# xuyuan/waymo_2d_tracking

Hardware: AMD Instinct MI355X
Metric: end-to-end frames/sec (detect+SORT) on 1920x1280 Waymo frames (higher is better)
Workload: dtype f32; 1 GPU; Cascade R-CNN X152-32x8d-FPN dconv (random-init, fp32, batch 1) on synthetic 1920x1280x3 frames -> top-100 detections/frame -> SORT (max_age 2, min_hits 0, all boxes tracked; trackers resident for the whole segment); 5 cameras x 2 frames per step per GPU; 1x1 and dense 3x3 convolutions: f32 operands as exact 3 x bf16 splits, six cross terms on the bf16 matrix cores, f32 accumulate (csrc/det_gemm_s; stage=e2e, parallelism=sequence-shard x1

## Files before the change

waymo_2d_tracking_amd/csrc/det_gemm_split.hip:

```cpp
#include "common.h"
#include "../../include/waymodet.h"
#include <cstdlib>
#include <cstring>

namespace {

using bf16x8 = __attribute__((ext_vector_type(8))) __bf16;
using bf16x2 = __attribute__((ext_vector_type(2))) __bf16;
using f32x2 = __attribute__((ext_vector_type(2))) float;
using f32x16 = __attribute__((ext_vector_type(16))) float;
using u32x4 = __attribute__((ext_vector_type(4))) unsigned;

constexpr int BK = 64;
constexpr int BN = 256;
constexpr int NTHREADS = 512;
constexpr int CHUNK = 6144;

struct SplitArgs {
    const float* a;
    const unsigned char* ap;
    const uint4* w;
    const float* bias;
    const float* residual;
    const unsigned char* resp;
    float* out;
    unsigned char* outp;
    long lda, ldc;
    int M, N, K, relu;
    int tiles_m, tiles_n;
    int splitk;
    float* part;
    long long* stamps;
    int H, W, C, Ho, Wo, stride, pad, ksize;
};

__device__ __forceinline__ unsigned pk_bf16(float a, float b) {
    const f32x2 v = {a, b};
    return __builtin_bit_cast(unsigned, __builtin_convertvector(v, bf16x2));
}

__device__ __forceinline__ void split_pair(float x0, float x1, unsigned& h, unsigned& m, unsigned& l) {
    h = pk_bf16(x0, x1);
    const float r0 = x0 - __uint_as_float(h << 16), r1 = x1 - __uint_as_float(h & 0xffff0000u);
    m = pk_bf16(r0, r1);
    const float s0 = r0 - __uint_as_float(m << 16), s1 = r1 - __uint_as_float(m & 0xffff0000u);
    l = pk_bf16(s0, s1);
}

__device__ __forceinline__ float bf_lo(unsigned v) { return __uint_as_float(v << 16); }
__device__ __forceinline__ float bf_hi(unsigned v) { return __uint_as_float(v & 0xffff0000u); }

__device__ __forceinline__ size_t planes_offset(int row, int col, int ncols) {
    return ((size_t)(row >> 5) * (size_t)(ncols >> 5) + (size_t)(col >> 5)) * CHUNK +
           (size_t)((row & 31) * 64 + ((((col >> 3) & 3) ^ ((row >> 2) & 3)) << 4) + ((col >> 2) & 1) * 8);
}

constexpr int LDC = BN + 8;

template <int MT>
__device__ __forceinline__ void split_epilogue(const SplitArgs& p, unsigned char* smem, const f32x16 (&acc)[MT], int m0, int n0, int wave, int lane, int mlim,
                                               int row_mul = 1, int row_add = 0) {
    const int rr = lane & 31, rg = lane >> 5;
    float* ct = reinterpret_cast<float*>(smem);
    const int ncols = p.N - n0 < BN ? p.N - n0 : BN;
    constexpr int PASS = 3;
    auto stage = [&](int i0) {
        if (i0 > 0) __builtin_amdgcn_s_barrier();
#pragma unroll
        for (int i = i0; i < i0 + PASS && i < MT; ++i)
#pragma unroll
            for (int e = 0; e < 16; ++e)
                ct[((i - i0) * 32 + (e & 3) + 8 * (e >> 2) + 4 * rg) * LDC + 32 * wave + rr] = acc[i][e];
        __builtin_amdgcn_s_waitcnt(0xC07F);
        __builtin_amdgcn_s_barrier();
    };
    if (p.outp == nullptr) {
        const int c4 = 4 * lane;
        float4 bv = make_float4(0.f, 0.f, 0.f, 0.f);
        if (p.bias && c4 < ncols) bv = *reinterpret_cast<const float4*>(p.bias + n0 + c4);
        constexpr int RPW = 32 * PASS / 8;
#pragma unroll
        for (int i0 = 0; i0 < MT; i0 += PASS) {
            const int nrows = 32 * ((MT - i0) < PASS ? (MT - i0) : PASS);
            float4 rv[RPW];
            if (p.residual) {
#pragma unroll
                for (int j = 0; j < RPW; ++j) {
                    const int r = wave + 8 * j, row = m0 + 32 * i0 + r;
                    rv[j] = make_float4(0.f, 0.f, 0.f, 0.f);
                    if (r < nrows && row < mlim && c4 < ncols)
                        rv[j] = *reinterpret_cast<const float4*>(p.residual + (size_t)(row * row_mul + row_add) * p.ldc + n0 + c4);
                }
            } else if (p.resp) {
#pragma unroll
                for (int j = 0; j < RPW; ++j) {
                    const int r = wave + 8 * j, row = m0 + 32 * i0 + r;
                    rv[j] = make_float4(0.f, 0.f, 0.f, 0.f);
                    if (r < nrows && row < mlim && c4 < ncols) {
                        const unsigned char* q = p.resp + planes_offset(row * row_mul + row_add, n0 + c4, p.N);
                        const uint2 h = *reinterpret_cast<const uint2*>(q), m = *reinterpret_cast<const uint2*>(q + 2048),
                                    l = *reinterpret_cast<const uint2*>(q + 4096);
                        rv[j] = make_float4((bf_lo(h.x) + bf_lo(m.x)) + bf_lo(l.x), (bf_hi(h.x) + bf_hi(m.x)) + bf_hi(l.x),
                                            (bf_lo(h.y) + bf_lo(m.y)) + bf_lo(l.y), (bf_hi(h.y) + bf_hi(m.y)) + bf_hi(l.y));
                    }
                }
            }
            stage(i0);
#pragma unroll
            for (int j = 0; j < RPW; ++j) {
                const int r = wave + 8 * j, row = m0 + 32 * i0 + r;
                if (r < nrows && row < mlim && c4 < ncols) {
                    float4 v = *reinterpret_cast<const float4*>(ct + r * LDC + c4);
                    v.x += bv.x; v.y += bv.y; v.z += bv.z; v.w += bv.w;
                    if (p.residual || p.resp) { v.x += rv[j].x; v.y += rv[j].y; v.z += rv[j].z; v.w += rv[j].w; }
                    if (p.relu) { v.x = fmaxf(v.x, 0.f); v.y = fmaxf(v.y, 0.f); v.z = fmaxf(v.z, 0.f); v.w = fmaxf(v.w, 0.f); }
                    *reinterpret_cast<float4*>(p.out + (size_t)(row * row_mul + row_add) * p.ldc + n0 + c4) = v;
                }
            }
        }
        return;
    }
    const int ur = lane >> 2;
    constexpr int UPW = PASS * 8 * 2 / 8;
    const int ncb = ncols >> 5;
#pragma unroll
    for (int i0 = 0; i0 < MT; i0 += PASS) {
        const int nrb = (MT - i0) < PASS ? (MT - i0) : PASS;
        const int nunits = nrb * ncb * 2;
        uint4 rq[UPW][3];
#pragma unroll
        for (int j = 0; j < UPW; ++j) {
            const int u = wave + 8 * j;
            rq[j][0] = rq[j][1] = rq[j][2] = make_uint4(0u, 0u, 0u, 0u);
            if (u < nunits && m0 + 32 * (i0 + u / (2 * ncb)) < mlim) {
                const int rbi = u / (2 * ncb), cb = (u >> 1) - rbi * ncb, h = u & 1;
                const int r = 16 * h + ur, row = m0 + 32 * (i0 + rbi) + r;
                const int c8 = 8 * ((lane & 3) ^ ((r >> 2) & 3)), col = n0 + 32 * cb + c8;
                if (p.resp) {
                    const unsigned char* q = p.resp + ((size_t)(row >> 5) * (size_t)(p.N >> 5) + (size_t)(col >> 5)) * CHUNK + h * 1024 + lane * 16;
                    rq[j][0] = *reinterpret_cast<const uint4*>(q);
                    rq[j][1] = *reinterpret_cast<const uint4*>(q + 2048);
                    rq[j][2] = *reinterpret_cast<const uint4*>(q + 4096);
                } else if (p.residual && row < mlim) {
                    const uint4* q = reinterpret_cast<const uint4*>(p.residual + (size_t)row * p.ldc + col);
                    rq[j][0] = q[0];
                    rq[j][1] = q[1];
                }
            }
        }
        stage(i0);
#pragma unroll
        for (int j = 0; j < UPW; ++j) {
            const int u = wave + 8 * j;
            if (u < nunits && m0 + 32 * (i0 + u / (2 * ncb)) < mlim) {
                const int rbi = u / (2 * ncb), cb = (u >> 1) - rbi * ncb, h = u & 1;
                const int r = 16 * h + ur, row = m0 + 32 * (i0 + rbi) + r;
                const int c8 = 8 * ((lane & 3) ^ ((r >> 2) & 3)), col = n0 + 32 * cb + c8;
                const float* src = ct + (32 * rbi + r) * LDC + 32 * cb + c8;
                float4 v0 = *reinterpret_cast<const float4*>(src), v1 = *reinterpret_cast<const float4*>(src + 4);
                if (p.bias) {
                    const float4 b0 = *reinterpret_cast<const float4*>(p.bias + col), b1 = *reinterpret_cast<const float4*>(p.bias + col + 4);
                    v0.x += b0.x; v0.y += b0.y; v0.z += b0.z; v0.w += b0.w; v1.x += b1.x; v1.y += b1.y; v1.z += b1.z; v1.w += b1.w;
                }
                if (p.resp) {
                    const uint4 hh = rq[j][0], mm = rq[j][1], ll = rq[j][2];
                    v0.x += (bf_lo(hh.x) + bf_lo(mm.x)) + bf_lo(ll.x); v0.y += (bf_hi(hh.x) + bf_hi(mm.x)) + bf_hi(ll.x);
                    v0.z += (bf_lo(hh.y) + bf_lo(mm.y)) + bf_lo(ll.y); v0.w += (bf_hi(hh.y) + bf_hi(mm.y)) + bf_hi(ll.y);
                    v1.x += (bf_lo(hh.z) + bf_lo(mm.z)) + bf_lo(ll.z); v1.y += (bf_hi(hh.z) + bf_hi(mm.z)) + bf_hi(ll.z);
                    v1.z += (bf_lo(hh.w) + bf_lo(mm.w)) + bf_lo(ll.w); v1.w += (bf_hi(hh.w) + bf_hi(mm.w)) + bf_hi(ll.w);
                } else if (p.residual) {
                    const uint4 q0 = rq[j][0], q1 = rq[j][1];
                    v0.x += __uint_as_float(q0.x); v0.y += __uint_as_float(q0.y); v0.z += __uint_as_float(q0.z); v0.w += __uint_as_float(q0.w);
                    v1.x += __uint_as_float(q1.x); v1.y += __uint_as_float(q1.y); v1.z += __uint_as_float(q1.z); v1.w += __uint_as_float(q1.w);
                }
                if (p.relu) {
                    v0.x = fmaxf(v0.x, 0.f); v0.y = fmaxf(v0.y, 0.f); v0.z = fmaxf(v0.z, 0.f); v0.w = fmaxf(v0.w, 0.f);
                    v1.x = fmaxf(v1.x, 0.f); v1.y = fmaxf(v1.y, 0.f); v1.z = fmaxf(v1.z, 0.f); v1.w = fmaxf(v1.w, 0.f);
                }
                if (p.out && row < mlim) {
                    float4* d = reinterpret_cast<float4*>(p.out + (size_t)row * p.ldc + col);
                    d[0] = v0; d[1] = v1;
                }
                unsigned hv[4], mv[4], lv[4];
                split_pair(v0.x, v0.y, hv[0], mv[0], lv[0]); split_pair(v0.z, v0.w, hv[1], mv[1], lv[1]);
                split_pair(v1.x, v1.y, hv[2], mv[2], lv[2]); split_pair(v1.z, v1.w, hv[3], mv[3], lv[3]);
                unsigned char* q = p.outp + ((size_t)(row >> 5) * (size_t)(p.N >> 5) + (size_t)(col >> 5)) * CHUNK + h * 1024 + lane * 16;
                *reinterpret_cast<uint4*>(q) = make_uint4(hv[0], hv[1], hv[2], hv[3]);
                *reinterpret_cast<uint4*>(q + 2048) = make_uint4(mv[0], mv[1], mv[2], mv[3]);
                *reinterpret_cast<uint4*>(q + 4096) = make_uint4(lv[0], lv[1], lv[2], lv[3]);
            }
        }
    }
}

__device__ __forceinline__ int xcd_tile_id(int total) {
    const int x = blockIdx.x & 7, j = blockIdx.x >> 3;
    const int q = total >> 3, r = total & 7;
    if (j >= q + (x < r ? 1 : 0)) return -1;
    return (x < r ? x * (q + 1) : r * (q + 1) + (x - r) * q) + j;
}

template <int MT, int MODE>
__global__ __launch_bounds__(NTHREADS, 2) void gemm_split_kernel(const SplitArgs p) {
    extern __shared__ __attribute__((aligned(16))) unsigned char smem[];
    constexpr int BM = 32 * MT;
    constexpr int PLANE = BM * 64;
    constexpr int BUF = 3 * PLANE;
    const int tid = threadIdx.x, lane = tid & 63;
    const int wave = __builtin_amdgcn_readfirstlane(tid >> 6);
    constexpr bool CONV = MODE == 1 || MODE == 3;
    constexpr bool PM = MODE == 3;
    int id = PM ? (int)blockIdx.x : xcd_tile_id(p.tiles_m * p.tiles_n * p.splitk);
    if (id < 0 || (PM && id >= p.tiles_m * p.tiles_n)) return;
#ifdef WD_DEBUG
    long long t_start = 0, r_start = 0, t_main = 0, t_epi = 0;
    if (p.stamps) { t_start = __builtin_amdgcn_s_memtime(); r_start = __builtin_amdgcn_s_memrealtime(); }
    const int id_stamp = id;
#endif
    const int kz = PM ? 0 : id % p.splitk;
    if (!PM) id /= p.splitk;
    const int tm = id / p.tiles_n, tn = id - tm * p.tiles_n;
    int m0 = tm * BM;
    const int n0 = tn * BN;
    const int kc = CONV ? p.C / 32 : 1;
    int pm_y = 0, pm_x = 0, pm_nvt = 9;
    unsigned long long pm_taps = 0x876543210ull;
    if (PM) {
        const int nch = (p.M / (p.H * p.W) + BM - 1) / BM;
        const int wi = p.W - 2, hi = p.H - 2, ni = wi * hi, ne = 2 * wi + 2 * hi;
        int t = tm, c, q;
        if (t < ni * nch) { c = t / ni; q = t - c * ni; pm_y = 1 + q / wi; pm_x = 1 + q - (q / wi) * wi; }
        else if (t < (ni + ne) * nch) {
            t -= ni * nch; c = t / ne; q = t - c * ne;
            if (q < wi) { pm_y = 0; pm_x = 1 + q; }
            else if (q < 2 * wi) { pm_y = p.H - 1; pm_x = 1 + q - wi; }
            else if (q < 2 * wi + hi) { pm_x = 0; pm_y = 1 + q - 2 * wi; }
            else { pm_x = p.W - 1; pm_y = 1 + q - 2 * wi - hi; }
        } else { t -= (ni + ne) * nch; c = t >> 2; q = t & 3; pm_y = (q >> 1) ? p.H - 1 : 0; pm_x = (q & 1) ? p.W - 1 : 0; }
        m0 = c * BM;
        pm_taps = 0; pm_nvt = 0;
        for (int tp = 0; tp < 9; ++tp) {
            const int yy = pm_y + tp / 3 - 1, xx = pm_x + tp % 3 - 1;
            if (yy >= 0 && yy < p.H && xx >= 0 && xx < p.W) { pm_taps |= (unsigned long long)tp << (4 * pm_nvt); ++pm_nvt; }
        }
    }
    auto pm_tap = [&](int i) { return (int)((pm_taps >> (4 * i)) & 15ull); };
    const int nk_all = PM ? pm_nvt * kc : p.K / 32;
    const int per = (nk_all + p.splitk - 1) / p.splitk;
    const int k0 = kz * per;
    const int nk = (k0 + per <= nk_all) ? per : nk_all - k0;

    const int srow = tid >> 4, sk2 = tid & 15;
    unsigned aoff[MT];
    unsigned vmask[MT];
#pragma unroll
    for (int i = 0; i < MT; ++i) {
        int m = m0 + srow + 32 * i;
        if (PM) {
            const int maps = p.M / (p.H * p.W);
            m = m < maps ? m : maps - 1;
            aoff[i] = (unsigned)(((m * p.H + pm_y - 1) * p.W + pm_x - 1) * p.C + 2 * sk2);
            vmask[i] = 0x1ffu;
            continue;
        }
        m = m < p.M ? m : p.M - 1;
        if (MODE == 0) {
            aoff[i] = (unsigned)(m * p.lda) + 2u * sk2;
            vmask[i] = 1u;
        } else {
            const int hw = p.Ho * p.Wo;
            const int b = m / hw, rem = m - b * hw;
            const int yo = rem / p.Wo, xo = rem - yo * p.Wo;
            const int y0 = yo * p.stride - p.pad, x0 = xo * p.stride - p.pad;
            aoff[i] = (unsigned)(((b * p.H + y0) * p.W + x0) * p.C + 2 * sk2);
            unsigned vm = 0;
            for (int t = 0; t < p.ksize * p.ksize; ++t) {
                const int yy = y0 + t / p.ksize, xx = x0 + t % p.ksize;
                if (yy >= 0 && yy < p.H && xx >= 0 && xx < p.W) vm |= 1u << t;
            }
            vmask[i] = vm;
        }
    }
    float2 araw[MT];
    auto a_fetch = [&](int kt, int i) -> float2 {
        kt = k0 + (kt < nk ? kt : nk - 1);
        if (MODE == 0) {
            return *reinterpret_cast<const float2*>(p.a + (size_t)(aoff[i] + (unsigned)(kt * 32)));
        } else {
            const int ti = kt / kc, cb = kt - ti * kc;
            const int tap = PM ? pm_tap(ti) : ti;
            const int dy = tap / p.ksize, dx = tap - dy * p.ksize;
            const unsigned delta = (unsigned)((dy * p.W + dx) * p.C + cb * 32);
            const bool ok = ((vmask[i] >> tap) & 1u) != 0;
            const unsigned off = ok ? aoff[i] + delta : 2u * sk2;
            const float2 v = *reinterpret_cast<const float2*>(p.a + (size_t)off);
            return ok ? v : make_float2(0.f, 0.f);
        }
    };
    auto a_load_row = [&](int kt, int i) { araw[i] = a_fetch(kt, i); };
    int f_idx = 0, f_tap = 0, f_cb = 0;
    unsigned f_delta = 0;
    int f_act = 0;
    auto f_place = [&]() {
        f_act = PM ? pm_tap(f_tap) : f_tap;
        const int dy = p.ksize == 3 ? (f_act * 11) >> 5 : 0, dx = f_act - dy * p.ksize;
        f_delta = (unsigned)((dy * p.W + dx) * p.C + f_cb * 32);
    };
    auto f_set = [&](int kt) {
        f_idx = kt < nk ? kt : nk - 1;
        const int ks = k0 + f_idx;
        f_tap = ks / kc; f_cb = ks - f_tap * kc;
        f_place();
    };
    auto f_advance = [&](int kt) {
        if (kt < nk && kt > f_idx) {
            ++f_idx;
            if (++f_cb == kc) { f_cb = 0; ++f_tap; }
            f_place();
        }
    };
    auto a_fetch_cur = [&](int i) -> float2 {
        const bool ok = ((vmask[i] >> f_act) & 1u) != 0;
        const unsigned off = ok ? aoff[i] + f_delta : 2u * sk2;
        const float2 v = *reinterpret_cast<const float2*>(p.a + (size_t)off);
        return ok ? v : make_float2(0.f, 0.f);
    };
    const int wofs = srow * 64 + ((((sk2 >> 2) ^ ((srow >> 2) & 3))) << 4) + ((sk2 & 3) << 2);
    auto a_store_val = [&](int bufoff, int i, float2 v) {
        unsigned char* base = smem + bufoff + wofs + i * 2048;
        unsigned h, m, l;
        split_pair(v.x, v.y, h, m, l);
        *reinterpret_cast<unsigned*>(base) = h;
        *reinterpret_cast<unsigned*>(base + PLANE) = m;
        *reinterpret_cast<unsigned*>(base + 2 * PLANE) = l;
    };
    auto a_store_row = [&](int bufoff, int i) { a_store_val(bufoff, i, araw[i]); };

    const int nt32 = (n0 >> 5) + wave;
    const bool active = nt32 * 32 < p.N;
    const uint4* wbase = p.w + (size_t)(active ? nt32 : 0) * (size_t)(p.K / 16) * 192 + lane;
    const int nsub = nk * 2;
    bf16x8 wf[2][3];
    auto w_load = [&](int sub, int slot) {
        sub = 2 * k0 + (sub < nsub ? sub : nsub - 1);
        if (PM) {
            const int ti = sub / (2 * kc);
            sub = pm_tap(ti) * 2 * kc + (sub - ti * 2 * kc);
        }
        const uint4* q = wbase + (size_t)sub * 192;
#pragma unroll
        for (int pl = 0; pl < 3; ++pl) wf[slot][pl] = __builtin_bit_cast(bf16x8, q[pl * 64]);
    };

    f32x16 acc[MT];
#pragma unroll
    for (int i = 0; i < MT; ++i)
#pragma unroll
        for (int e = 0; e < 16; ++e) acc[i][e] = 0.f;

    const int rr = lane & 31, rg = lane >> 5;
    const int rofs0 = rr * 64 + ((((0 + rg) ^ ((rr >> 2) & 3))) << 4);
    const int rofs1 = rr * 64 + ((((2 + rg) ^ ((rr >> 2) & 3))) << 4);

    {
        float2 p0[MT], p1[MT];
#pragma unroll
        for (int i = 0; i < MT; ++i) p0[i] = a_fetch(0, i);
        w_load(0, 0);
        w_load(1, 1);
#pragma unroll
        for (int i = 0; i < MT; ++i) p1[i] = a_fetch(1, i);
#pragma unroll
        for (int i = 0; i < MT; ++i) a_load_row(2, i);
#pragma unroll
        for (int i = 0; i < MT; ++i) a_store_val(0, i, p0[i]);
#pragma unroll
        for (int i = 0; i < MT; ++i) a_store_val(BUF, i, p1[i]);
    }
    float2 aahead[MT];
#pragma unroll
    for (int i = 0; i < MT; ++i) aahead[i] = a_fetch(3, i);
#ifdef WD_DEBUG
    if (p.stamps) t_main = __builtin_amdgcn_s_memtime();
#endif
    __builtin_amdgcn_s_waitcnt(0xC07F);
    __builtin_amdgcn_s_barrier();

    bf16x8 af[MT][3];
#define SB __builtin_amdgcn_sched_barrier(0)
#define MF(pa, pb, slot)                                                                                      \
    _Pragma("unroll") for (int i = 0; i < MT; ++i)                                                          \
        acc[i] = __builtin_amdgcn_mfma_f32_32x32x16_bf16(af[i][pa], wf[slot][pb], acc[i], 0, 0, 0);
#define RD(addr, pl)                                                                                          \
    _Pragma("unroll") for (int i = 0; i < MT; ++i)                                                          \
        af[i][pl] = *reinterpret_cast<const bf16x8*>(smem + (addr) + (pl) * PLANE + i * 2048);
#define SPLIT_ROW(i_)                                                                                         \
    if ((i_) < MT) { a_store_row(wr, (i_)); araw[(i_)] = aahead[(i_)]; aahead[(i_)] = CONV ? a_fetch_cur((i_)) : a_fetch(kt + 4, (i_)); }
    RD(rofs0, 2) RD(rofs0, 1) RD(rofs0, 0)
    SB;
    int cur = 0, nxt = BUF, wr = 2 * BUF;
    if (CONV) f_set(4);
    for (int kt = 0; kt < nk; ++kt) {
        const int a1 = cur + rofs1, a0n = nxt + rofs0;
        MF(2, 0, 0) RD(a1, 2) SB;
        MF(1, 1, 0) SPLIT_ROW(0) SB;
        MF(1, 0, 0) RD(a1, 1) SB;
        MF(0, 2, 0) SPLIT_ROW(1) SB;
        MF(0, 1, 0) SPLIT_ROW(2) SB;
        MF(0, 0, 0) RD(a1, 0) w_load(2 * kt + 2, 0); SB;
        MF(2, 0, 1) RD(a0n, 2) SB;
        MF(1, 1, 1) SPLIT_ROW(3) SB;
        MF(1, 0, 1) RD(a0n, 1) SB;
        MF(0, 2, 1) SPLIT_ROW(4) SB;
        MF(0, 1, 1) SPLIT_ROW(5) SB;
        MF(0, 0, 1) RD(a0n, 0) w_load(2 * kt + 3, 1); SB;
        __builtin_amdgcn_s_waitcnt(0xC07F | (MT << 8));
        __builtin_amdgcn_s_barrier();
        SB;
        const int t = cur; cur = nxt; nxt = wr; wr = t;
        if (CONV) f_advance(kt + 5);
    }
#undef SPLIT_ROW
#ifdef WD_DEBUG
    if (p.stamps) t_epi = __builtin_amdgcn_s_memtime();
#endif
    __builtin_amdgcn_s_waitcnt(0xC07F);
    __builtin_amdgcn_s_barrier();
    if (p.splitk > 1) {
        SplitArgs q = p;
        q.out = p.part + (size_t)kz * p.M * p.N;
        q.ldc = p.N;
        q.bias = nullptr; q.residual = nullptr; q.resp = nullptr; q.outp = nullptr; q.relu = 0;
        split_epilogue<MT>(q, smem, acc, m0, n0, wave, lane, p.M);
    } else if (PM) {
        split_epilogue<MT>(p, smem, acc, m0, n0, wave, lane, p.M / (p.H * p.W), p.H * p.W, pm_y * p.W + pm_x);
    } else {
        split_epilogue<MT>(p, smem, acc, m0, n0, wave, lane, p.M);
    }
#ifdef WD_DEBUG
    if (p.stamps && tid == 0) {
        long long* o = p.stamps + 8 * (long)blockIdx.x;
        o[0] = t_start; o[1] = t_main; o[2] = t_epi; o[3] = __builtin_amdgcn_s_memtime();
        o[4] = id_stamp; o[5] = __builtin_amdgcn_s_getreg(20  | (0 << 6) | (3 << 11));
        o[6] = r_start; o[7] = __builtin_amdgcn_s_memrealtime();
    }
#endif
}

#undef MF
#undef RD

template <int MT>
__global__ __launch_bounds__(NTHREADS, 2) void gemm_split_planes_kernel(const SplitArgs p) {
    extern __shared__ __attribute__((aligned(16))) unsigned char smem[];
    constexpr int BM = 32 * MT;
    constexpr int PLANE = BM * 64;
    constexpr int BUF = 3 * PLANE;
    constexpr int NPIECE = 6 * MT;
    constexpr int ND = (NPIECE + 7) / 8;
    const int tid = threadIdx.x, lane = tid & 63;
    const int wave = __builtin_amdgcn_readfirstlane(tid >> 6);
    int id = xcd_tile_id(p.tiles_m * p.tiles_n * p.splitk);
    if (id < 0) return;
#ifdef WD_DEBUG
    long long t_start = 0, r_start = 0, t_main = 0, t_epi = 0;
    if (p.stamps) { t_start = __builtin_amdgcn_s_memtime(); r_start = __builtin_amdgcn_s_memrealtime(); }
    const int id_stamp = id;
#endif
    const int kz = id % p.splitk;
    id /= p.splitk;
    const int tm = id / p.tiles_n, tn = id - tm * p.tiles_n;
    const int m0 = tm * BM, n0 = tn * BN;
    const int nk_all = p.K / 32;
    const int per = (nk_all + p.splitk - 1) / p.splitk;
    const int k0 = kz * per;
    const int nk = (k0 + per <= nk_all) ? per : nk_all - k0;

    const int nrb = (p.M + 31) >> 5;
    const size_t rb_stride = (size_t)nk_all * CHUNK;
    const unsigned char* dsrc[ND];
    unsigned ddst[ND];
#pragma unroll
    for (int j = 0; j < ND; ++j) {
        int c = wave + 8 * j;
        c = c < NPIECE ? c : NPIECE - 1;
        const int i = c / 6, pl = (c - 6 * i) >> 1, h = c & 1;
        int rb = tm * MT + i;
        rb = rb < nrb ? rb : nrb - 1;
        dsrc[j] = p.ap + (size_t)rb * rb_stride + (size_t)k0 * CHUNK + pl * 2048 + h * 1024;
        ddst[j] = (unsigned)(pl * PLANE + i * 2048 + h * 1024);
    }
    const unsigned lane16 = (unsigned)lane * 16u;
    auto dma16 = [&](const unsigned char* sbase, unsigned dst) {
        unsigned keep;
        asm volatile("s_mov_b32 %0, m0\n\ts_mov_b32 m0, %3\n\ts_nop 0\n\tglobal_load_lds_dwordx4 %1, %2\n\ts_mov_b32 m0, %0"
                     : "=&s"(keep) : "v"(lane16), "s"(sbase), "s"(dst) : "memory");
    };
    auto dma_piece = [&](int kt, unsigned bufoff, int j) {
        kt = kt < nk ? kt : nk - 1;
        dma16(dsrc[j] + (size_t)kt * CHUNK, bufoff + ddst[j]);
    };

    const int nt32 = (n0 >> 5) + wave;
    const bool active = nt32 * 32 < p.N;
    const unsigned char* wbase = reinterpret_cast<const unsigned char*>(p.w + (size_t)(active ? nt32 : 0) * (size_t)(p.K / 16) * 192);
    const int nsub = nk * 2;
    u32x4 wf[2][3];
    auto w_load = [&](int sub, int slot) {
        sub = 2 * k0 + (sub < nsub ? sub : nsub - 1);
        const unsigned char* q = wbase + (size_t)sub * 3072;
        asm volatile("global_load_dwordx4 %0, %3, %4\n\tglobal_load_dwordx4 %1, %3, %4 offset:1024\n\tglobal_load_dwordx4 %2, %3, %4 offset:2048"
                     : "=&v"(wf[slot][0]), "=&v"(wf[slot][1]), "=&v"(wf[slot][2]) : "v"(lane16), "s"(q) : "memory");
    };
#define WAITW(slot, n) asm volatile("s_waitcnt vmcnt(%3)" : "+v"(wf[slot][0]), "+v"(wf[slot][1]), "+v"(wf[slot][2]) : "n"(n) : "memory")

    f32x16 acc[MT];
#pragma unroll
    for (int i = 0; i < MT; ++i)
#pragma unroll
        for (int e = 0; e < 16; ++e) acc[i][e] = 0.f;

    const int rr = lane & 31, rg = lane >> 5;
    const int rofs0 = rr * 64 + ((((0 + rg) ^ ((rr >> 2) & 3))) << 4);
    const int rofs1 = rr * 64 + ((((2 + rg) ^ ((rr >> 2) & 3))) << 4);

#pragma unroll
    for (int s = 0; s < 3; ++s)
#pragma unroll
        for (int j = 0; j < ND; ++j) dma_piece(s, (unsigned)(s * BUF), j);
    w_load(0, 0);
    w_load(1, 1);
#ifdef WD_DEBUG
    if (p.stamps) t_main = __builtin_amdgcn_s_memtime();
#endif
    asm volatile("s_waitcnt vmcnt(0)" : "+v"(wf[0][0]), "+v"(wf[0][1]), "+v"(wf[0][2]), "+v"(wf[1][0]), "+v"(wf[1][1]), "+v"(wf[1][2]) :: "memory");
    __builtin_amdgcn_s_barrier();

    bf16x8 af[MT][3];
#define SB __builtin_amdgcn_sched_barrier(0)
#define MF(pa, pb, slot)                                                                                      \
    _Pragma("unroll") for (int i = 0; i < MT; ++i)                                                          \
        acc[i] = __builtin_amdgcn_mfma_f32_32x32x16_bf16(af[i][pa], __builtin_bit_cast(bf16x8, wf[slot][pb]), acc[i], 0, 0, 0);
#define RD(addr, pl)                                                                                          \
    _Pragma("unroll") for (int i = 0; i < MT; ++i)                                                          \
        af[i][pl] = *reinterpret_cast<const bf16x8*>(smem + (addr) + (pl) * PLANE + i * 2048);
#define DMA(j_)                                                                                               \
    if ((j_) < ND) { dma_piece(kt + 3, (unsigned)wr, (j_)); }
    RD(rofs0, 2) RD(rofs0, 1) RD(rofs0, 0)
    SB;
    int cur = 0, nxt = BUF, nx2 = 2 * BUF, wr = 3 * BUF;
    for (int kt = 0; kt < nk; ++kt) {
        const int a1 = cur + rofs1, a0n = nxt + rofs0;
        WAITW(0, ND + 3);
        MF(2, 0, 0) RD(a1, 2) SB;
        MF(1, 1, 0) SB;
        MF(1, 0, 0) RD(a1, 1) SB;
        MF(0, 2, 0) SB;
        MF(0, 1, 0) SB;
        MF(0, 0, 0) RD(a1, 0) w_load(2 * kt + 2, 0); SB;
        WAITW(1, 3);
        MF(2, 0, 1) RD(a0n, 2) SB;
        MF(1, 1, 1) DMA(0) DMA(3) SB;
        MF(1, 0, 1) RD(a0n, 1) SB;
        MF(0, 2, 1) DMA(1) DMA(4) SB;
        MF(0, 1, 1) DMA(2) SB;
        MF(0, 0, 1) RD(a0n, 0) w_load(2 * kt + 3, 1); SB;
        __builtin_amdgcn_s_barrier();
        SB;
        const int t = cur; cur = nxt; nxt = nx2; nx2 = wr; wr = t;
    }
#undef DMA
#undef WAITW
#ifdef WD_DEBUG
    if (p.stamps) t_epi = __builtin_amdgcn_s_memtime();
#endif
    asm volatile("s_waitcnt vmcnt(0) lgkmcnt(0)" ::: "memory");
    __builtin_amdgcn_s_barrier();
    if (p.splitk > 1) {
        SplitArgs q = p;
        q.out = p.part + (size_t)kz * p.M * p.N;
        q.ldc = p.N;
        q.bias = nullptr; q.residual = nullptr; q.resp = nullptr; q.outp = nullptr; q.relu = 0;
        split_epilogue<MT>(q, smem, acc, m0, n0, wave, lane, p.M);
    } else {
        split_epilogue<MT>(p, smem, acc, m0, n0, wave, lane, p.M);
    }
#ifdef WD_DEBUG
    if (p.stamps && tid == 0) {
        long long* o = p.stamps + 8 * (long)blockIdx.x;
        o[0] = t_start; o[1] = t_main; o[2] = t_epi; o[3] = __builtin_amdgcn_s_memtime();
        o[4] = id_stamp; o[5] = __builtin_amdgcn_s_getreg(20  | (0 << 6) | (3 << 11));
        o[6] = r_start; o[7] = __builtin_amdgcn_s_memrealtime();
    }
#endif
}
#undef SB
#undef MF
#undef RD

__global__ __launch_bounds__(256) void split_planes_pack_kernel(const float* __restrict__ a, long lda, int M, int K, unsigned char* __restrict__ out, long total) {
    const long t = (long)blockIdx.x * 256 + threadIdx.x;
    if (t >= total) return;
    const int k8 = K / 8;
    const int row = (int)(t / k8), kq = (int)(t - (long)row * k8);
    float4 v0 = make_float4(0.f, 0.f, 0.f, 0.f), v1 = v0;
    if (row < M) {
        const float4* s = reinterpret_cast<const float4*>(a + (size_t)row * lda + 8 * kq);
        v0 = s[0]; v1 = s[1];
    }
    unsigned h[4], m[4], l[4];
    split_pair(v0.x, v0.y, h[0], m[0], l[0]); split_pair(v0.z, v0.w, h[1], m[1], l[1]);
    split_pair(v1.x, v1.y, h[2], m[2], l[2]); split_pair(v1.z, v1.w, h[3], m[3], l[3]);
    unsigned char* q = out + planes_offset(row, 8 * kq, K);
    *reinterpret_cast<uint4*>(q) = make_uint4(h[0], h[1], h[2], h[3]);
    *reinterpret_cast<uint4*>(q + 2048) = make_uint4(m[0], m[1], m[2], m[3]);
    *reinterpret_cast<uint4*>(q + 4096) = make_uint4(l[0], l[1], l[2], l[3]);
}

__global__ __launch_bounds__(256) void split_planes_unpack_kernel(const unsigned char* __restrict__ planes, int M, int K, float* __restrict__ out, long ldo, long total) {
    const long t = (long)blockIdx.x * 256 + threadIdx.x;
    if (t >= total) return;
    const int k8 = K / 8;
    const int row = (int)(t / k8), kq = (int)(t - (long)row * k8);
    const unsigned char* q = planes + planes_offset(row, 8 * kq, K);
    const uint4 h = *reinterpret_cast<const uint4*>(q), m = *reinterpret_cast<const uint4*>(q + 2048), l = *reinterpret_cast<const uint4*>(q + 4096);
    float4* d = reinterpret_cast<float4*>(out + (size_t)row * ldo + 8 * kq);
    d[0] = make_float4((bf_lo(h.x) + bf_lo(m.x)) + bf_lo(l.x), (bf_hi(h.x) + bf_hi(m.x)) + bf_hi(l.x), (bf_lo(h.y) + bf_lo(m.y)) + bf_lo(l.y),
                       (bf_hi(h.y) + bf_hi(m.y)) + bf_hi(l.y));
    d[1] = make_float4((bf_lo(h.z) + bf_lo(m.z)) + bf_lo(l.z), (bf_hi(h.z) + bf_hi(m.z)) + bf_hi(l.z), (bf_lo(h.w) + bf_lo(m.w)) + bf_lo(l.w),
                       (bf_hi(h.w) + bf_hi(m.w)) + bf_hi(l.w));
}

__global__ __launch_bounds__(256) void gemm_split_pack_kernel(const float* __restrict__ w, int N, int K, long sn, long sk, uint4* __restrict__ out, long total) {
    const long t = (long)blockIdx.x * 256 + threadIdx.x;
    if (t >= total) return;
    const int k8 = K / 8;
    const int n = (int)(t / k8), kq = (int)(t - (long)n * k8);
    float v[8];
#pragma unroll
    for (int e = 0; e < 8; ++e) v[e] = n < N ? w[(size_t)n * sn + (size_t)(8 * kq + e) * sk] : 0.f;
    unsigned h[4], m[4], l[4];
#pragma unroll
    for (int e = 0; e < 4; ++e) split_pair(v[2 * e], v[2 * e + 1], h[e], m[e], l[e]);
    const int nt = n >> 5, ks = kq >> 1, ln = (n & 31) + 32 * (kq & 1);
    uint4* dst = out + ((size_t)nt * (K / 16) + ks) * 192 + ln;
    dst[0] = make_uint4(h[0], h[1], h[2], h[3]);
    dst[64] = make_uint4(m[0], m[1], m[2], m[3]);
    dst[128] = make_uint4(l[0], l[1], l[2], l[3]);
}

__global__ __launch_bounds__(256) void gemm_split_pack_batch_kernel(const WdSplitPackDesc* __restrict__ descs, int count) {
    int lo = 0, hi = count - 1;
    const long blk = blockIdx.x;
    while (lo < hi) {
        const int mid = (lo + hi + 1) >> 1;
        if (descs[mid].first_block <= blk) lo = mid; else hi = mid - 1;
    }
    const WdSplitPackDesc d = descs[lo];
    const long t = (blk - d.first_block) * 256 + threadIdx.x;
    const int k8 = d.K / 8;
    const long total = (long)((d.N + 31) / 32) * 32 * k8;
    if (t >= total) return;
    const int n = (int)(t / k8), kq = (int)(t - (long)n * k8);
    const int k = 8 * kq, tap = k / d.C, c = k - tap * d.C;
    int kh = tap / d.ksize, kw = tap - kh * d.ksize;
    if (d.flip) { kh = d.ksize - 1 - kh; kw = d.ksize - 1 - kw; }
    const float* src = d.src + (size_t)n * d.s_n + (size_t)kh * d.s_kh + (size_t)kw * d.s_kw + (size_t)c * d.s_c;
    float v[8];
#pragma unroll
    for (int e = 0; e < 8; ++e) v[e] = n < d.N ? src[(size_t)e * d.s_c] : 0.f;
    unsigned h[4], m[4], l[4];
#pragma unroll
    for (int e = 0; e < 4; ++e) split_pair(v[2 * e], v[2 * e + 1], h[e], m[e], l[e]);
    const int nt = n >> 5, ks = kq >> 1, ln = (n & 31) + 32 * (kq & 1);
    uint4* dst = reinterpret_cast<uint4*>(d.dst) + ((size_t)nt * (d.K / 16) + ks) * 192 + ln;
    dst[0] = make_uint4(h[0], h[1], h[2], h[3]);
    dst[64] = make_uint4(m[0], m[1], m[2], m[3]);
    dst[128] = make_uint4(l[0], l[1], l[2], l[3]);
}

__global__ __launch_bounds__(256) void gemm_split_reduce_kernel(const float4* __restrict__ part, int splitk, long mn4, int n4, const float4* __restrict__ bias,
                                                                const float* __restrict__ residual, const unsigned char* __restrict__ resp, long ldc, int relu,
                                                                float* __restrict__ out, unsigned char* __restrict__ outp) {
    const long i = (long)blockIdx.x * 256 + threadIdx.x;
    if (i >= mn4) return;
    float4 v = part[i];
    for (int z = 1; z < splitk; ++z) {
        const float4 q = part[(size_t)z * mn4 + i];
        v.x += q.x; v.y += q.y; v.z += q.z; v.w += q.w;
    }
    const long row = i / n4;
    const int c4 = (int)(i - row * n4);
    if (bias) { const float4 b = bias[c4]; v.x += b.x; v.y += b.y; v.z += b.z; v.w += b.w; }
    const size_t o = (size_t)row * ldc + 4 * c4;
    if (residual) { const float4 q = *reinterpret_cast<const float4*>(residual + o); v.x += q.x; v.y += q.y; v.z += q.z; v.w += q.w; }
    if (resp) {
        const unsigned char* q = resp + planes_offset((int)row, 4 * c4, 4 * n4);
        const uint2 h = *reinterpret_cast<const uint2*>(q), m = *reinterpret_cast<const uint2*>(q + 2048), l = *reinterpret_cast<const uint2*>(q + 4096);
        v.x += (bf_lo(h.x) + bf_lo(m.x)) + bf_lo(l.x); v.y += (bf_hi(h.x) + bf_hi(m.x)) + bf_hi(l.x);
        v.z += (bf_lo(h.y) + bf_lo(m.y)) + bf_lo(l.y); v.w += (bf_hi(h.y) + bf_hi(m.y)) + bf_hi(l.y);
    }
    if (relu) { v.x = fmaxf(v.x, 0.f); v.y = fmaxf(v.y, 0.f); v.z = fmaxf(v.z, 0.f); v.w = fmaxf(v.w, 0.f); }
    if (out) *reinterpret_cast<float4*>(out + o) = v;
    if (outp) {
        unsigned h0, m0_, l0, h1, m1, l1;
        split_pair(v.x, v.y, h0, m0_, l0);
        split_pair(v.z, v.w, h1, m1, l1);
        unsigned char* q = outp + planes_offset((int)row, 4 * c4, 4 * n4);
        *reinterpret_cast<uint2*>(q) = make_uint2(h0, h1);
        *reinterpret_cast<uint2*>(q + 2048) = make_uint2(m0_, m1);
        *reinterpret_cast<uint2*>(q + 4096) = make_uint2(l0, l1);
    }
}

bool experiment_mode() {
    static const bool on = []() { const char* e = getenv("WT_EXPERIMENT"); return e && e[0] == '1'; }();
    return on;
}
int experiment_knob(const char* name) {
    const char* e = getenv(name);
    if (!e) return 0;
    if (!experiment_mode()) {
        fprintf(stderr, "libwaymotrack: %s=%s ignored (laboratory switch; set WT_EXPERIMENT=1 to use it)\n", name, e);
        return 0;
    }
// ... 282 lines not shown
```

Before: 42.69 frames/s.

## Stage A tile with float4 loads in wide units and defer conv zero-padding

```diff
diff --git a/waymo_2d_tracking_amd/csrc/det_gemm_split.hip b/waymo_2d_tracking_amd/csrc/det_gemm_split.hip
--- a/waymo_2d_tracking_amd/csrc/det_gemm_split.hip
+++ b/waymo_2d_tracking_amd/csrc/det_gemm_split.hip
@@ -200,6 +200,47 @@
     return (x < r ? x * (q + 1) : r * (q + 1) + (x - r) * q) + j;
 }
 
+constexpr int stage_units(int mt) { return (mt + 1) / 2; }
+constexpr bool stage_wide(int mt, int u) { return u < mt / 2; }
+constexpr int stage_row0(int mt, int u) { return stage_wide(mt, u) ? 64 * u : 32 * (mt - 1); }
+constexpr int stage_row(bool wide, int row0, int tid) { return row0 + (wide ? tid >> 3 : tid >> 4); }
+constexpr int stage_col(bool wide, int tid) { return wide ? 4 * (tid & 7) : 2 * (tid & 15); }
+constexpr int stage_offset(bool wide, int row0, int tid) {
+    const int r = stage_row(wide, row0, tid);
+    if (wide) { const int q = tid & 7; return r * 64 + (((q >> 1) ^ ((r >> 2) & 3)) << 4) + ((q & 1) << 3); }
+    const int s = tid & 15;
+    return r * 64 + (((s >> 2) ^ ((r >> 2) & 3)) << 4) + ((s & 3) << 2);
+}
+constexpr int stage_pair_byte(int r, int s) {
+    const int srow = r & 31;
+    return srow * 64 + (((s >> 2) ^ ((srow >> 2) & 3)) << 4) + ((s & 3) << 2) + (r >> 5) * 2048;
+}
+constexpr bool stage_covers(int mt) {
+    int hits[32 * 6 * 16] = {};
+    for (int u = 0; u < stage_units(mt); ++u) {
+        const bool wide = stage_wide(mt, u);
+        for (int tid = 0; tid < NTHREADS; ++tid) {
+            const int r = stage_row(wide, stage_row0(mt, u), tid), s = stage_col(wide, tid) / 2, off = stage_offset(wide, stage_row0(mt, u), tid);
+            if (r < 0 || r >= 32 * mt || (off & (wide ? 7 : 3))) return false;
+            for (int e = 0; e < (wide ? 2 : 1); ++e) {
+                if (off + 4 * e != stage_pair_byte(r, s + e)) return false;
+                ++hits[r * 16 + s + e];
+            }
+        }
+    }
+    for (int i = 0; i < 32 * mt * 16; ++i)
+        if (hits[i] != 1) return false;
+    return true;
+}
+static_assert(stage_covers(2) && stage_covers(3) && stage_covers(4) && stage_covers(5) && stage_covers(6),
+              "A staging units must write every (row, float pair) of a K step once, at the byte of the fragment layout");
+
+constexpr int stage_slot(int mt, int pos) {
+    const int nu = stage_units(mt);
+    const int u = nu <= 2 ? (pos == 1 ? 0 : pos == 4 ? 1 : -1) : (pos == 1 ? 0 : pos == 3 ? 1 : pos == 4 ? 2 : -1);
+    return u < nu ? u : -1;
+}
+
 template <int MT, int MODE>
 __global__ __launch_bounds__(NTHREADS, 2) void gemm_split_kernel(const SplitArgs p) {
     extern __shared__ __attribute__((aligned(16))) unsigned char smem[];
@@ -250,54 +291,62 @@
     const int k0 = kz * per;
     const int nk = (k0 + per <= nk_all) ? per : nk_all - k0;
 
-    const int srow = tid >> 4, sk2 = tid & 15;
-    unsigned aoff[MT];
-    unsigned vmask[MT];
-#pragma unroll
-    for (int i = 0; i < MT; ++i) {
-        int m = m0 + srow + 32 * i;
+    constexpr int NU = stage_units(MT);
+    auto u_wide = [](int u) { return stage_wide(MT, u); };
+    auto u_col = [&](int u) { return (unsigned)stage_col(u_wide(u), tid); };
+    unsigned aoff[NU];
+    unsigned vmask[NU];
+#pragma unroll
+    for (int u = 0; u < NU; ++u) {
+        int m = m0 + stage_row(u_wide(u), stage_row0(MT, u), tid);
         if (PM) {
             const int maps = p.M / (p.H * p.W);
             m = m < maps ? m : maps - 1;
-            aoff[i] = (unsigned)(((m * p.H + pm_y - 1) * p.W + pm_x - 1) * p.C + 2 * sk2);
-            vmask[i] = 0x1ffu;
+            aoff[u] = (unsigned)(((m * p.H + pm_y - 1) * p.W + pm_x - 1) * p.C) + u_col(u);
+            vmask[u] = 0x1ffu;
             continue;
         }
         m = m < p.M ? m : p.M - 1;
         if (MODE == 0) {
-            aoff[i] = (unsigned)(m * p.lda) + 2u * sk2;
-            vmask[i] = 1u;
+            aoff[u] = (unsigned)(m * p.lda) + u_col(u);
+            vmask[u] = 1u;
         } else {
             const int hw = p.Ho * p.Wo;
             const int b = m / hw, rem = m - b * hw;
             const int yo = rem / p.Wo, xo = rem - yo * p.Wo;
             const int y0 = yo * p.stride - p.pad, x0 = xo * p.stride - p.pad;
-            aoff[i] = (unsigned)(((b * p.H + y0) * p.W + x0) * p.C + 2 * sk2);
+            aoff[u] = (unsigned)(((b * p.H + y0) * p.W + x0) * p.C) + u_col(u);
             unsigned vm = 0;
             for (int t = 0; t < p.ksize * p.ksize; ++t) {
                 const int yy = y0 + t / p.ksize, xx = x0 + t % p.ksize;
                 if (yy >= 0 && yy < p.H && xx >= 0 && xx < p.W) vm |= 1u << t;
             }
-            vmask[i] = vm;
-        }
-    }
-    float2 araw[MT];
-    auto a_fetch = [&](int kt, int i) -> float2 {
+            vmask[u] = vm;
+        }
+    }
+    auto a_ld = [&](unsigned off, int u) -> float4 {
+        if (u_wide(u)) return *reinterpret_cast<const float4*>(p.a + (size_t)off);
+        const float2 v = *reinterpret_cast<const float2*>(p.a + (size_t)off);
+        return make_float4(v.x, v.y, 0.f, 0.f);
+    };
+    const float4 zero4 = make_float4(0.f, 0.f, 0.f, 0.f);
+    float4 araw[NU];
+    constexpr bool ZERO_PAD = CONV && !PM;
+    auto a_fetch = [&](int kt, int u, bool zero_now = true) -> float4 {
         kt = k0 + (kt < nk ? kt : nk - 1);
         if (MODE == 0) {
-            return *reinterpret_cast<const float2*>(p.a + (size_t)(aoff[i] + (unsigned)(kt * 32)));
+            return a_ld(aoff[u] + (unsigned)(kt * 32), u);
         } else {
             const int ti = kt / kc, cb = kt - ti * kc;
             const int tap = PM ? pm_tap(ti) : ti;
             const int dy = tap / p.ksize, dx = tap - dy * p.ksize;
             const unsigned delta = (unsigned)((dy * p.W + dx) * p.C + cb * 32);
-            const bool ok = ((vmask[i] >> tap) & 1u) != 0;
-            const unsigned off = ok ? aoff[i] + delta : 2u * sk2;
-            const float2 v = *reinterpret_cast<const float2*>(p.a + (size_t)off);
-            return ok ? v : make_float2(0.f, 0.f);
-        }
-    };
-    auto a_load_row = [&](int kt, int i) { araw[i] = a_fetch(kt, i); };
+            const bool ok = PM || ((vmask[u] >> tap) & 1u) != 0;
+            const unsigned off = ok ? aoff[u] + delta : u_col(u);
+            const float4 v = a_ld(off, u);
+            return (ok || !zero_now) ? v : zero4;
+        }
+    };
     int f_idx = 0, f_tap = 0, f_cb = 0;
     unsigned f_delta = 0;
     int f_act = 0;
@@ -319,33 +368,39 @@
             f_place();
         }
     };
-    auto a_fetch_cur = [&](int i) -> float2 {
-        const bool ok = ((vmask[i] >> f_act) & 1u) != 0;
-        const unsigned off = ok ? aoff[i] + f_delta : 2u * sk2;
-        const float2 v = *reinterpret_cast<const float2*>(p.a + (size_t)off);
-        return ok ? v : make_float2(0.f, 0.f);
-    };
-    const int wofs = srow * 64 + ((((sk2 >> 2) ^ ((srow >> 2) & 3))) << 4) + ((sk2 & 3) << 2);
-    auto a_store_val = [&](int bufoff, int i, float2 v) {
-        unsigned char* base = smem + bufoff + wofs + i * 2048;
-        unsigned h, m, l;
-        split_pair(v.x, v.y, h, m, l);
-        *reinterpret_cast<unsigned*>(base) = h;
-        *reinterpret_cast<unsigned*>(base + PLANE) = m;
-        *reinterpret_cast<unsigned*>(base + 2 * PLANE) = l;
-    };
-    auto a_store_row = [&](int bufoff, int i) { a_store_val(bufoff, i, araw[i]); };
+    auto a_fetch_cur = [&](int u) -> float4 {
+        const bool ok = PM || ((vmask[u] >> f_act) & 1u) != 0;
+        return a_ld(ok ? aoff[u] + f_delta : u_col(u), u);
+    };
+    auto tap_of = [&](int kt) { return (k0 + (kt < nk ? kt : nk - 1)) / kc; };
+    int s_act0 = ZERO_PAD ? tap_of(2) : 0, s_act1 = ZERO_PAD ? tap_of(3) : 0;
+    auto a_store_val = [&](int bufoff, int u, float4 v) {
+        unsigned char* base = smem + bufoff + stage_offset(u_wide(u), stage_row0(MT, u), tid);
+        unsigned s0[3], s1[3] = {0u, 0u, 0u};
+        split_pair(v.x, v.y, s0[0], s0[1], s0[2]);
+        if (u_wide(u)) split_pair(v.z, v.w, s1[0], s1[1], s1[2]);
+#pragma unroll
+        for (int pl = 0; pl < 3; ++pl) {
+            if (u_wide(u)) *reinterpret_cast<uint2*>(base + pl * PLANE) = make_uint2(s0[pl], s1[pl]);
+            else *reinterpret_cast<unsigned*>(base + pl * PLANE) = s0[pl];
+        }
+    };
 
     const int nt32 = (n0 >> 5) + wave;
     const bool active = nt32 * 32 < p.N;
     const uint4* wbase = p.w + (size_t)(active ? nt32 : 0) * (size_t)(p.K / 16) * 192 + lane;
     const int nsub = nk * 2;
     bf16x8 wf[2][3];
+    int w_idx = 0, w_ti = 0, w_rest = 0, w_sub = PM ? pm_tap(0) * 2 * kc : 0;
     auto w_load = [&](int sub, int slot) {
-        sub = 2 * k0 + (sub < nsub ? sub : nsub - 1);
         if (PM) {
-            const int ti = sub / (2 * kc);
-            sub = pm_tap(ti) * 2 * kc + (sub - ti * 2 * kc);
+            if (sub < nsub && sub > w_idx) {
+                ++w_idx; ++w_sub;
+                if (++w_rest == 2 * kc) { w_rest = 0; ++w_ti; w_sub = pm_tap(w_ti) * 2 * kc; }
+            }
+            sub = w_sub;
+        } else {
+            sub = 2 * k0 + (sub < nsub ? sub : nsub - 1);
         }
         const uint4* q = wbase + (size_t)sub * 192;
 #pragma unroll
@@ -363,23 +418,23 @@
     const int rofs1 = rr * 64 + ((((2 + rg) ^ ((rr >> 2) & 3))) << 4);
 
     {
-        float2 p0[MT], p1[MT];
-#pragma unroll
-        for (int i = 0; i < MT; ++i) p0[i] = a_fetch(0, i);
+        float4 p0[NU], p1[NU];
+#pragma unroll
+        for (int u = 0; u < NU; ++u) p0[u] = a_fetch(0, u);
         w_load(0, 0);
         w_load(1, 1);
 #pragma unroll
-        for (int i = 0; i < MT; ++i) p1[i] = a_fetch(1, i);
-#pragma unroll
-        for (int i = 0; i < MT; ++i) a_load_row(2, i);
-#pragma unroll
-        for (int i = 0; i < MT; ++i) a_store_val(0, i, p0[i]);
-#pragma unroll
-        for (int i = 0; i < MT; ++i) a_store_val(BUF, i, p1[i]);
-    }
-    float2 aahead[MT];
-#pragma unroll
-    for (int i = 0; i < MT; ++i) aahead[i] = a_fetch(3, i);
+        for (int u = 0; u < NU; ++u) p1[u] = a_fetch(1, u);
+#pragma unroll
+        for (int u = 0; u < NU; ++u) araw[u] = a_fetch(2, u, !ZERO_PAD);
+#pragma unroll
+        for (int u = 0; u < NU; ++u) a_store_val(0, u, p0[u]);
+#pragma unroll
+        for (int u = 0; u < NU; ++u) a_store_val(BUF, u, p1[u]);
+    }
+    float4 aahead[NU];
+#pragma unroll
+    for (int u = 0; u < NU; ++u) aahead[u] = a_fetch(3, u, !ZERO_PAD);
 #ifdef WD_DEBUG
     if (p.stamps) t_main = __builtin_amdgcn_s_memtime();
 #endif
@@ -394,8 +449,18 @@
 #define RD(addr, pl)                                                                                          \
     _Pragma("unroll") for (int i = 0; i < MT; ++i)                                                          \
         af[i][pl] = *reinterpret_cast<const bf16x8*>(smem + (addr) + (pl) * PLANE + i * 2048);
-#define SPLIT_ROW(i_)                                                                                         \
-    if ((i_) < MT) { a_store_row(wr, (i_)); araw[(i_)] = aahead[(i_)]; aahead[(i_)] = CONV ? a_fetch_cur((i_)) : a_fetch(kt + 4, (i_)); }
+    auto stage_unit = [&](int u, int kt, int bufoff) {
+        float4 v = araw[u];
+        araw[u] = aahead[u];
+        aahead[u] = CONV ? a_fetch_cur(u) : a_fetch(kt + 4, u);
+        if (ZERO_PAD && ((vmask[u] >> s_act0) & 1u) == 0) v = zero4;
+        a_store_val(bufoff, u, v);
+    };
+#define STAGE(pos_)                                                                                           \
+    {                                                                                                         \
+        constexpr int u_ = stage_slot(MT, (pos_));                                                            \
+        if constexpr (u_ >= 0) stage_unit(u_, kt, wr);                                                        \
+    }
     RD(rofs0, 2) RD(rofs0, 1) RD(rofs0, 0)
     SB;
     int cur = 0, nxt = BUF, wr = 2 * BUF;
@@ -403,24 +468,25 @@
     for (int kt = 0; kt < nk; ++kt) {
         const int a1 = cur + rofs1, a0n = nxt + rofs0;
         MF(2, 0, 0) RD(a1, 2) SB;
-        MF(1, 1, 0) SPLIT_ROW(0) SB;
+        MF(1, 1, 0) STAGE(0) SB;
         MF(1, 0, 0) RD(a1, 1) SB;
-        MF(0, 2, 0) SPLIT_ROW(1) SB;
-        MF(0, 1, 0) SPLIT_ROW(2) SB;
+        MF(0, 2, 0) STAGE(1) SB;
+        MF(0, 1, 0) STAGE(2) SB;
         MF(0, 0, 0) RD(a1, 0) w_load(2 * kt + 2, 0); SB;
         MF(2, 0, 1) RD(a0n, 2) SB;
-        MF(1, 1, 1) SPLIT_ROW(3) SB;
+        MF(1, 1, 1) STAGE(3) SB;
         MF(1, 0, 1) RD(a0n, 1) SB;
-        MF(0, 2, 1) SPLIT_ROW(4) SB;
-        MF(0, 1, 1) SPLIT_ROW(5) SB;
+        MF(0, 2, 1) STAGE(4) SB;
+        MF(0, 1, 1) STAGE(5) SB;
         MF(0, 0, 1) RD(a0n, 0) w_load(2 * kt + 3, 1); SB;
         __builtin_amdgcn_s_waitcnt(0xC07F | (MT << 8));
         __builtin_amdgcn_s_barrier();
         SB;
         const int t = cur; cur = nxt; nxt = wr; wr = t;
+        if (ZERO_PAD) { s_act0 = s_act1; s_act1 = f_act; }
         if (CONV) f_advance(kt + 5);
     }
-#undef SPLIT_ROW
+#undef STAGE
 #ifdef WD_DEBUG
     if (p.stamps) t_epi = __builtin_amdgcn_s_memtime();
 #endif
```

New measurement: 43.03 frames/s, median of 6. Within noise of the previous version (+0.8%).
